# SuperbTUM/Multimodal-ReID

Hardware: AMD Instinct MI355X
Metric: gallery imgs/sec + eval wall-sec (distmat+rerank); mAP parity Market/MSMT17 (higher is better)
Workload: dtype fp16; 1 GPU; Market-1501 full eval: 3368q x 15913g, ViT-B/16 stride-12 (211 tokens), 2 passes/img (plain + flip/pad/crop TTA), exact-fp32 distmat, CMC/mAP; batch=20480, images_per_encoder_call=19281, parallelism=dp1 (image shards + all-gather)

## Files before the change

### include/reidmi_tools.h

```cpp
#ifndef REIDMI_TOOLS_H
#define REIDMI_TOOLS_H
#include "reidmi.h"

#ifdef __cplusplus
extern "C" {
#endif

int reidmi_distmat_f32_variant(const float* q, int64_t Q, int64_t ldq, const float* g, int64_t G, int64_t ldg,
                               int64_t D, float* out, int64_t ldo, float* ws, int variant, void* stream);

int64_t reidmi_search_ex_workspace_bytes(int64_t Q, int64_t G, int64_t D, int k, int splits, int cap);
int reidmi_search_f32_ex(const float* q, int64_t Q, int64_t ldq, const float* g, int64_t G, int64_t ldg, int64_t D,
                         int k, const int64_t* q_pids, const int64_t* q_cams, const int64_t* g_pids,
                         const int64_t* g_cams, int32_t* out_idx, float* out_dist, int64_t ldo, void* ws,
                         int64_t ws_bytes, int splits, int cap, int32_t* stats, void* stream);
int reidmi_search_bounded_f32_ex(const float* q, int64_t Q, int64_t ldq, const float* g, int64_t G, int64_t ldg,
                                 int64_t D, int k, const int64_t* q_pids, const int64_t* q_cams,
                                 const int64_t* g_pids, const int64_t* g_cams, const float* bound_dist,
                                 const int32_t* bound_idx, int64_t ldb, int64_t index_base, int32_t* out_idx,
                                 float* out_dist, int64_t ldo, void* ws, int64_t ws_bytes, int splits, int cap,
                                 int32_t* stats, void* stream);

int reidmi_gemm_f16_tiled(int epi, const void* A, int64_t lda, const void* W, int64_t ldw, int64_t M, int64_t N,
                          int64_t K, const float* bias, const void* rowstat, const float* colsum, void* out,
                          int64_t ldc, int tile, int ngroups, void* stream);

int reidmi_gemm_f16_w4(const void* A, int64_t lda, const void* W, int64_t ldw, int64_t M, int64_t N, int64_t K,
                       const float* bias, void* out, int64_t ldc, int nostore, void* stream);

int reidmi_mhsa_f16_rr(const void* q, const void* k, const void* vt, void* o, int64_t nseq, int L, int H,
                       void* stream);

int reidmi_mhsa_cls_f16(const void* q, const void* k, const void* vt, void* o, int64_t nseq, int L, int H,
                        void* stream);

int reidmi_mhsa_cls_long_f16(const void* q, const void* k, const void* vt, void* o, int64_t nseq, int L, int H,
                             void* stream);

int64_t reidmi_cls_attn_nokv_ws_bytes(int64_t nseq, int W);
int reidmi_cls_attn_nokv_f16(const void* x, const void* rs, const void* q, const void* wqkv, const float* colsum,
// ... 30 lines not shown
```

### multimodal-reid_amd/csrc/encoder.hip

```cpp
#include "attention.h"
#include "gemm.h"

namespace reidmi {

template <typename TX>
__device__ __forceinline__ float4 load4(const TX* p) {
    if constexpr (sizeof(TX) == 4) {
        return *(const float4*)p;
    } else {
        const f16x4 h = *(const f16x4*)p;
        return make_float4((float)h[0], (float)h[1], (float)h[2], (float)h[3]);
    }
}

template <int NV, typename TX>
__global__ __launch_bounds__(256) void layernorm_kernel(const TX* x, int64_t rows, int64_t ldx,
                                                        const int32_t* __restrict__ row_idx,
                                                        const float* __restrict__ gamma,
                                                        const float* __restrict__ beta, float eps,
                                                        float* __restrict__ y32, int64_t ldy32,
                                                        _Float16* __restrict__ y16, int64_t ldy16,
                                                        _Float16* yh, int64_t ldyh, float2* __restrict__ st,
                                                        float2* __restrict__ sto) {
    const int64_t r = (int64_t)blockIdx.x * 4 + (threadIdx.x >> 6);
// ... 369 lines not shown
    int64_t x, h, q, k, vt, o, u, rows, st, st_cls, pst, total;
};

static int64_t al(int64_t v) { return (v + 255) & ~(int64_t)255; }

static Plan plan(int64_t nseq, int L, int W, int lp, int64_t extra_rows) {
    Plan p{};
    const int64_t M = nseq * L;
    int64_t off = 0;
    p.x = off; off = al(off + M * W * 2);
    p.h = off; off = al(off + M * W * 2);
    p.q = off; off = al(off + M * W * 2);
    p.k = off; off = al(off + M * W * 2);
    p.vt = off; off = al(off + nseq * W * (int64_t)lp * 2);
    p.o = off; off = al(off + M * W * 2);
    p.u = off; off = al(off + M * 4 * W * 2);
    p.rows = off; off = al(off + extra_rows * 4);
    p.st = off; off = al(off + (M + 256) * 8);
    p.st_cls = off; off = al(off + (nseq + 256) * 8);
    p.pst = off; off = al(off + M * (W / 64) * 8);
    p.total = off;
    return p;
}

enum XStats { XS_ROWS = 0, XS_PARTIALS = 1, XS_READY = 2 };

static int ln1_stats(XStats xs, char* ws, const Plan& P, int64_t M, int W, hipStream_t s) {
    float2* st = (float2*)(ws + P.st);
    if (xs == XS_READY) return OK;
    if (xs == XS_PARTIALS) return row_stats_from_partials((const float2*)(ws + P.pst), M, W, st, s);
    return row_stats((const _Float16*)(ws + P.x), M, W, W, st, s);
}

static int run_block(const reidmi_block_weights& bw, char* ws, const Plan& P, int64_t nseq, int L, int W, int H,
                     bool causal, XStats xs, hipStream_t s) {
    const int64_t M = nseq * L;
    float2* pst = (float2*)(ws + P.pst);
    _Float16* x = (_Float16*)(ws + P.x);
    _Float16* o = (_Float16*)(ws + P.o);
    _Float16* u = (_Float16*)(ws + P.u);
    float2* st = (float2*)(ws + P.st);
    int rc;
    if ((rc = ln1_stats(xs, ws, P, M, W, s))) return rc;
    {
        EpiArgs ea{};
        ea.bias = bw.qkv_b;
        ea.rowstat = st;
        ea.colsum = bw.qkv_s;
        ea.q = ws + P.q;
        ea.k = ws + P.k;
        ea.vt = ws + P.vt;
// ... 5 lines not shown
    }
    EpiArgs er{};
    er.out = x;
    er.ldc = W;
    er.bias = bw.out_b;
    er.pstat = pst;
    er.ldp = M;
    if ((rc = gemm_f16(EPI_RESID_F16, o, W, bw.out_w, W, M, W, W, er, s))) return rc;
    if ((rc = row_stats_from_partials(pst, M, W, st, s))) return rc;
    EpiArgs eg{};
    eg.out = u;
    eg.ldc = 4 * W;
    eg.bias = bw.fc1_b;
    eg.rowstat = st;
    eg.colsum = bw.fc1_s;
    if ((rc = gemm_f16(EPI_GELU_H16, x, W, bw.fc1_w, W, M, 4 * W, W, eg, s))) return rc;
    EpiArgs e2{};
    e2.out = x;
    e2.ldc = W;
    e2.bias = bw.fc2_b;
    e2.pstat = pst;
    e2.ldp = M;
    if ((rc = gemm_f16(EPI_RESID_F16, u, 4 * W, bw.fc2_w, 4 * W, M, W, 4 * W, e2, s))) return rc;
    return OK;
}

__global__ void gather_rowstat_kernel(const float2* __restrict__ st, int64_t nseq, int L, float2* __restrict__ sc) {
    const int64_t b = (int64_t)blockIdx.x * blockDim.x + threadIdx.x;
    if (b < nseq) sc[b] = st[b * L];
}

static int run_block_cls(const reidmi_block_weights& bw, char* ws, const Plan& P, int64_t nseq, int L, int W, int H,
                         XStats xs, hipStream_t s) {
    const int64_t M = nseq * L;
    _Float16* x = (_Float16*)(ws + P.x);
    _Float16* o = (_Float16*)(ws + P.o);
    _Float16* u = (_Float16*)(ws + P.u);
    float2* st = (float2*)(ws + P.st);
// ... 69 lines not shown

REIDMI_API int reidmi_layernorm(const float* x, int64_t rows, int64_t ldx, const int32_t* row_idx, int64_t W,
                                const float* gamma, const float* beta, float eps, float* y32, int64_t ldy32, void* y16,
                                int64_t ldy16, void* stream) {
    return layernorm(x, rows, ldx, row_idx, W, gamma, beta, eps, y32, ldy32, (_Float16*)y16, ldy16,
                     (hipStream_t)stream);
}

REIDMI_API int64_t reidmi_vit_workspace_bytes(const reidmi_vit_weights* w, int64_t B, int full) {
    if (vit_check(w)) return -1;
    const int64_t L = 1 + (int64_t)w->grid_h * w->grid_w + w->n_ctx;
    if (L < 1 || L > kAttnLongMax) return -1;
    return plan(B, (int)L, w->width, attn_vt_stride((int)L), 0).total;
}

REIDMI_API int reidmi_vit_forward(const reidmi_vit_weights* w, const void* images, int images_f16, int64_t B, int H,
                                  int Wimg, const int32_t* tta, int full, float* out_x12, float* out_proj,
                                  float* out_x11, void* ws_, int64_t ws_bytes, void* stream) {
    int rc;
    if ((rc = vit_check(w))) return rc;
    hipStream_t s = (hipStream_t)stream;
    RM_REQUIRE(1 + (int64_t)w->grid_h * w->grid_w + w->n_ctx <= 1024, "vit: too many tokens (max 1024)");
    const int W = w->width, NP = w->grid_h * w->grid_w, L = 1 + NP + w->n_ctx, E = w->out_dim;
    RM_REQUIRE((H - w->patch) / w->stride + 1 == w->grid_h && (Wimg - w->patch) / w->stride + 1 == w->grid_w,
               "vit: image size does not match the positional-embedding grid");
    const Plan P = plan(B, L, W, attn_vt_stride(L), 0);
    RM_REQUIRE(ws_bytes >= P.total, "vit: workspace too small");
    RM_REQUIRE(out_x12 && out_proj, "vit: outputs required");
    if (B == 0) return OK;
    char* ws = (char*)ws_;
    _Float16* x = (_Float16*)(ws + P.x);
    _Float16* h = (_Float16*)(ws + P.h);
    _Float16* col = (_Float16*)(ws + P.u);
    const int64_t M = B * L;
    if ((rc = im2col(images, images_f16, B, H, Wimg, w->patch, w->stride, w->grid_h, w->grid_w, w->kpad, tta, col, s)))
        return rc;
    if ((rc = patch_embed(col, w->conv_w, w->pos_emb, w->class_emb, w->vpt, w->n_ctx, B, NP, W, w->kpad, x, s)))
        return rc;
    if ((rc = layernorm(x, M, W, nullptr, W, w->ln_pre_w, w->ln_pre_b, 1e-5f, nullptr, 0, nullptr, 0, s, x, W, nullptr,
                        (float2*)(ws + P.st))))
        return rc;
    for (int i = 0; i < 12; i++) {
        const reidmi_block_weights& bw = w->blocks[i];
        if (i > 0 && bw.prompt && w->n_ctx > 0) {
            const int64_t pe = B * w->n_ctx * W;
            hipLaunchKernelGGL(prompt_rows_kernel, dim3(ceil_div(pe, 256)), dim3(256), 0, s, x, B, L, W,
                               L - w->n_ctx, w->n_ctx, bw.prompt);
            RM_LAUNCHED();
        }
        const XStats xs = i == 0 ? XS_READY : (bw.prompt && w->n_ctx > 0) ? XS_ROWS : XS_PARTIALS;
        if (i == 11 && !full) rc = run_block_cls(bw, ws, P, B, L, W, w->heads, xs, s);
        else rc = run_block(bw, ws, P, B, L, W, w->heads, false, xs, s);
        if (rc) return rc;
        if (i == 10 && out_x11) {
            const int64_t r11 = full ? M : B;
            hipLaunchKernelGGL(rows_f16_to_f32_kernel, dim3(ceil_div(r11 * (W / 4), 256)), dim3(256), 0, s, x, r11,
                               full ? (int64_t)W : (int64_t)L * W, W, out_x11);
            RM_LAUNCHED();
        }
    }
    const int64_t rows = full ? M : B;
    const int64_t ldx = full ? W : (int64_t)L * W;
    if ((rc = layernorm(x, rows, ldx, nullptr, W, w->ln_post_w, w->ln_post_b, 1e-5f, out_x12, W, h, W, s))) return rc;
    EpiArgs eo{};
    eo.out = out_proj;
    eo.ldc = E;
    if ((rc = gemm_f16(EPI_F32, h, W, w->proj_t, W, rows, E, W, eo, s))) return rc;
    return OK;
}

REIDMI_API int64_t reidmi_text_workspace_bytes(const reidmi_text_weights* w, int64_t N) {
    if (!w || attn_lpad(w->ctx) < 0) return -1;
    return plan(N, w->ctx, w->width, attn_lpad(w->ctx), N).total;
}

REIDMI_API int reidmi_text_forward(const reidmi_text_weights* w, const int64_t* tokens, const float* prompts,
                                   int64_t N, int ctx_used, float* out, void* ws_, int64_t ws_bytes, void* stream) {
    RM_REQUIRE(w && w->blocks && tokens && out, "text: null argument");
    RM_REQUIRE(w->width == w->heads * 64 && w->width % 256 == 0, "text: width");
    hipStream_t s = (hipStream_t)stream;
    const int W = w->width, Lt = w->ctx, E = w->out_dim;
    const int L = ctx_used > 0 ? ctx_used : Lt;
    RM_REQUIRE(L <= Lt && L > w->n_ctx, "text: ctx_used must be in (n_ctx, ctx]");
    RM_REQUIRE(attn_lpad(L) > 0, "text: context too long");
    const Plan P = plan(N, L, W, attn_lpad(L), N);
    RM_REQUIRE(ws_bytes >= P.total, "text: workspace too small");
    if (N == 0) return OK;
    char* ws = (char*)ws_;
    _Float16* x = (_Float16*)(ws + P.x);
    _Float16* h = (_Float16*)(ws + P.h);
    int32_t* rows = (int32_t*)(ws + P.rows);
    int rc;
    if ((rc = text_embed(x, tokens, prompts, w->tok_emb, w->pos_emb, N, L, Lt, W, (int64_t)w->vocab, s))) return rc;
    for (int i = 0; i < w->layers; i++) {
        const reidmi_block_weights& bw = w->blocks[i];
        if (i > 0 && bw.prompt && w->n_ctx > 0) {
            const int64_t pe = N * w->n_ctx * W;
            hipLaunchKernelGGL(prompt_rows_kernel, dim3(ceil_div(pe, 256)), dim3(256), 0, s, x, N, L, W, 1,
                               w->n_ctx, bw.prompt);
            RM_LAUNCHED();
        }
        const XStats xs = i > 0 && !(bw.prompt && w->n_ctx > 0) ? XS_PARTIALS : XS_ROWS;
        if ((rc = run_block(bw, ws, P, N, L, W, w->heads, true, xs, s))) return rc;
    }
    if ((rc = eot_rows(tokens, N, L, Lt, rows, s))) return rc;
    if ((rc = layernorm(x, N, W, rows, W, w->ln_final_w, w->ln_final_b, 1e-5f, nullptr, 0, h, W, s))) return rc;
    EpiArgs eo{};
    eo.out = out;
// ... 11 lines not shown
REIDMI_API int reidmi_gemm_f16_resid_partials(const void* A, int64_t lda, const void* Wt, int64_t ldw, int64_t M,
                                              int64_t N, int64_t K, const float* bias, void* out, int64_t ldc,
                                              void* pst, void* stream) {
    RM_REQUIRE(A && Wt && out && pst && N % 64 == 0, "resid partials: null argument or N % 64 != 0");
    EpiArgs e{};
    e.out = out;
    e.ldc = ldc;
    e.bias = bias;
    e.pstat = (float2*)pst;
    e.ldp = M;
    return gemm_f16(EPI_RESID_F16, (const _Float16*)A, lda, (const _Float16*)Wt, ldw, M, (int)N, (int)K, e,
                    (hipStream_t)stream);
}

#ifdef REIDMI_TOOLS
REIDMI_API int reidmi_im2col_f16(const void* images, int images_f16, int64_t B, int H, int Wimg, int patch, int stride,
                                 int gh, int gw, int kpad, const int32_t* tta, void* col, void* stream) {
    RM_REQUIRE(images && col && B >= 0 && H > 0 && Wimg > 0, "im2col: null argument or bad shape");
    return im2col(images, images_f16, B, H, Wimg, patch, stride, gh, gw, kpad, tta, (_Float16*)col,
                  (hipStream_t)stream);
}

REIDMI_API int reidmi_patch_embed_f16(const void* col, const void* conv_w, const float* pos_emb,
                                      const float* class_emb, const float* vpt, int n_ctx, int64_t B, int NP, int W,
                                      int kpad, void* x, int tile, void* stream) {
    RM_REQUIRE(col && conv_w && pos_emb && class_emb && x && n_ctx >= 0 && B >= 0 && NP > 0 && W > 0,
               "patch_embed: null argument or bad shape");
    if (B == 0) return OK;
    GemmOpts opt;
    opt.tile = tile;
// ... 25 lines not shown
```

### multimodal-reid_amd/csrc/gemm.h

```cpp
#pragma once
#include "common.h"

namespace reidmi {

enum Epi : int {
    EPI_H16 = 0,
    EPI_GELU_H16 = 1,
    EPI_QKV = 3,
    EPI_PATCH = 4,
    EPI_F32 = 5,
    EPI_RESID_F16 = 6,
    EPI_RRHI = 7,
    EPI_RRSV = 8
};

struct EpiArgs {
    void* out;
    int64_t ldc;
    const float* bias;
    void* q;
    void* k;
    void* vt;
    int seq;
    int heads;
// ... 11 lines not shown
    int64_t rr_n;
    float rr_c[3];
    const float* rr_csqn;
    const float* rr_cnrm;
    const float4* rr_rowmeta;
    const float4* rr_colrec;
    const int* rr_tiles;
    int64_t rr_ntiles;
    int rr_tri;
    int* sv_cnt;
    int2* sv_list;
    int sv_cap;
    const float* dist_rsq;
    const float* dist_csq;
    int64_t dist_n;
};

__device__ __forceinline__ float rr_hi(float dot, float si, float sj, float crn_i, float ni, float nj,
                                       const float (&c)[3]) {
    const float s = si + sj;
    const float dt = __builtin_fmaf(-2.0f, dot, s);
    const float e = 1.01f * (__builtin_fmaf(crn_i, nj, 0x1p-23f * s) + c[1] * (ni + nj) + c[2]);
    return dt + e;
}

struct GemmOpts {
    int tile = 0;
    int ngroups = 0;
    int band = -1;
};

int gemm_f16(int epi, const void* A, int64_t lda, const void* W, int64_t ldw, int64_t M, int64_t N, int64_t K,
             const EpiArgs& ea, hipStream_t stream, const GemmOpts& opts = GemmOpts{});

int gemm_api(int epi, const void* A, int64_t lda, const void* W, int64_t ldw, int64_t M, int64_t N, int64_t K,
             const float* bias, const void* rowstat, const float* colsum, void* out, int64_t ldc, const GemmOpts& opt,
             void* stream);

int prof_begin(double flops, int epi, hipStream_t s, hipEvent_t* end);
int prof_end(hipEvent_t end, hipStream_t s);

}
```

### multimodal-reid_amd/csrc/gemm.hip

```cpp
#include "gemm_epilogue.h"
#include "gemm_rrsv.h"
#include <type_traits>

namespace reidmi {

template <int EPI>
__global__ __launch_bounds__(256, 2) void gemm_tile_kernel(const _Float16* __restrict__ A, int64_t lda,
                                                           const _Float16* __restrict__ W, int64_t ldw, int64_t M,
                                                           int N, int K, EpiArgs ea, int tiles_n, int nwg) {
    __shared__ __attribute__((aligned(16))) _Float16 smem[2][2][GB_M * GB_K];
    const int bid = blockIdx.x;
    const int xcd = bid & 7, qq = nwg >> 3, rr = nwg & 7;
    const int wg = (xcd < rr ? xcd * (qq + 1) : rr * (qq + 1) + (xcd - rr) * qq) + (bid >> 3);
    const int tm = wg / tiles_n, tn = wg % tiles_n;
    const int64_t m0 = (int64_t)tm * GB_M;
    const int n0 = tn * GB_N;
    const int tid = threadIdx.x, lane = tid & 63, wid = tid >> 6;
    const int wm = wid >> 1, wn = wid & 1;

    const _Float16* gA[4];
    const _Float16* gW[4];
    int soff[4];
    bool aval[4];
#pragma unroll
// ... 66 lines not shown
        const int cq = (lane >> 4) * 4;
#pragma unroll
        for (int j = 0; j < 4; j++)
            bn[j] = ea.bias ? *(const float4*)(ea.bias + n0 + wn * 64 + j * 16 + cq) : make_float4(0.f, 0.f, 0.f, 0.f);
        ln_fold<4>(acc, ea.rowstat, ea.colsum, bn, m0 + wm * 64, n0 + wn * 64, M);
        epilogue_tile<EPI, 4, true>(ea, acc, m0 + wm * 64, n0 + wn * 64, M, N);
        return;
    }
    epilogue_tile<EPI, 4>(ea, acc, m0 + wm * 64, n0 + wn * 64, M, N);
#undef GLOAD
#undef LSTORE
}

constexpr int G2_STAGE = (G2_M + G2_N) * GB_K;

template <int EPI, int TAG = 0>
__global__ __launch_bounds__(512, 2) void gemm_persistent_kernel(const _Float16* __restrict__ A, int64_t lda,
                                                                 const _Float16* __restrict__ W, int64_t ldw,
                                                                 int64_t M, int N, int K, EpiArgs ea, int tiles_m,
                                                                 int tiles_n, int ngroups, int band) {
    extern __shared__ __attribute__((aligned(16))) _Float16 lds[];
    const int G = gridDim.x;
    const int bid = blockIdx.x;
    const int ng = G < 8 ? G : 8;
    const int xg = bid % ng, gx = G / ng + ((G % ng) > xg ? 1 : 0);
    const int ngr = (ng == 8 && 8 % ngroups == 0 && ngroups <= tiles_n) ? ngroups : 1;
    const int xper = ng / ngr, grp = xg / xper, xs = xg - grp * xper;
    const int nb0 = tiles_n * grp / ngr, tnk = tiles_n * (grp + 1) / ngr - nb0;
    const int64_t sub = (int64_t)tiles_m * tnk;
    const int lo = (int)(sub * xs / xper), hi = (int)(sub * (xs + 1) / xper);
    const int first = lo + bid / ng;
    if (first >= hi) return;
    if constexpr (EPI == EPI_RESID_F16) {
        if (bid & 1) __builtin_amdgcn_s_sleep(127);
    }
    const int tid = threadIdx.x, lane = tid & 63;
    const int wid = __builtin_amdgcn_readfirstlane(tid >> 6);
    const int wr = wid >> 2, wc = wid & 3;
    const int nk = K / GB_K;

    int rowA[2][2], kcA[2][2], offA[2][2], offW[2][2];
    uint32_t offAb[2][2], offWb[2][2];
#pragma unroll
    for (int h = 0; h < 2; h++)
#pragma unroll
        for (int u = 0; u < 2; u++) {
            const int pc = 2 * wid + u;
            const int ra = 128 * (pc >> 3) + 64 * h + 8 * (pc & 7);
            const int rb = 64 * (pc >> 2) + 32 * h + 8 * (pc & 3);
            const int r1 = ra + (lane >> 3), r2 = rb + (lane >> 3);
            rowA[h][u] = r1;
            kcA[h][u] = ((lane & 7) ^ ((r1 >> 1) & 7)) * 8;
            offAb[h][u] = (uint32_t)(r1 * (int)lda + kcA[h][u]) * 2u;
            offWb[h][u] = (uint32_t)(r2 * (int)ldw + ((lane & 7) ^ ((r2 >> 1) & 7)) * 8) * 2u;
            offA[h][u] = ra * GB_K;
            offW[h][u] = G2_M * GB_K + rb * GB_K;
        }
    const int* const rr_list = EPI == EPI_RRSV ? ea.rr_tiles : nullptr;
    if constexpr (EPI != EPI_RRHI) band = 0;
    struct Pos {
        int tile, kt;
        int64_t m0;
        int n0;
        bool full;
        const char* a;
        const char* w;
    };
    auto set_tile = [&](Pos& p, int tile) {
        p.tile = tile;
        p.kt = 0;
        int mt, nt;
        tile_mn<EPI == EPI_RRSV>(tile, tnk, band, tiles_m, rr_list, mt, nt);
        p.m0 = (int64_t)mt * G2_M;
        p.n0 = (nb0 + nt) * G2_N;
        p.full = p.m0 + G2_M <= M;
        p.a = (const char*)(A + (GEMM_VAR_ASAME ? 0 : p.m0) * lda);
        p.w = (const char*)(W + (int64_t)p.n0 * ldw);
    };
    auto advance = [&](Pos& p) {
        if (++p.kt == nk) {
            set_tile(p, p.tile + gx);
        } else {
            p.a += GB_K * 2;
            p.w += GB_K * 2;
        }
    };
    auto issue_a = [&](int stage, int h, const Pos& p) {
        const char* base = p.a;
        if (p.full) {
#pragma unroll
            for (int u = 0; u < 2; u++)
                __builtin_amdgcn_global_load_lds(base + offAb[h][u],
                                                 (lds_ptr_t)(lds + stage * G2_STAGE + offA[h][u]), 16, 0, 0);
        } else {
            const int lim = (int)(M - p.m0);
#pragma unroll
            for (int u = 0; u < 2; u++) {
                const int r = rowA[h][u] < lim ? rowA[h][u] : lim - 1;
                __builtin_amdgcn_global_load_lds(base + (uint32_t)(r * (int)lda + kcA[h][u]) * 2u,
                                                 (lds_ptr_t)(lds + stage * G2_STAGE + offA[h][u]), 16, 0, 0);
            }
        }
    };
    auto issue_w = [&](int stage, int h, const Pos& p) {
// ... 212 lines not shown
#pragma unroll
            for (int i = 0; i < 8; i++)
#pragma unroll
                for (int j = 0; j < 4; j++) {
                    acc[i][j][0] = __builtin_fmaf(rs[i].x, acc[i][j][0], __builtin_fmaf(rs[i].y, sn[j].x, b[j].x));
                    acc[i][j][1] = __builtin_fmaf(rs[i].x, acc[i][j][1], __builtin_fmaf(rs[i].y, sn[j].y, b[j].y));
                    acc[i][j][2] = __builtin_fmaf(rs[i].x, acc[i][j][2], __builtin_fmaf(rs[i].y, sn[j].z, b[j].z));
                    acc[i][j][3] = __builtin_fmaf(rs[i].x, acc[i][j][3], __builtin_fmaf(rs[i].y, sn[j].w, b[j].w));
                }
        }
        if constexpr (EPI == EPI_RRSV)
            rrsv_tile(ea, acc, m0 + wr * 128, n0 + wc * 64, M, seq, ea.rr_tri && tmt < tnt, rr_lds + (seq & 1) * 4096,
                      rr_lds + 8192 + (seq & 1) * 4096, sv_lds, sv_n, lane,
                      RrsvWalk{first, gx, wr, wc, rr_list});
        else if (EPI == EPI_GELU_H16 && m0 + G2_M <= M)
            epilogue_tile<EPI, 8, true, RPRE, true>(ea, acc, m0 + wr * 128, n0 + wc * 64, M, N, xres);
        else
            epilogue_tile<EPI, 8, true, RPRE>(ea, acc, m0 + wr * 128, n0 + wc * 64, M, N, xres);
        seq++;
        if (wr == 1) G5_BARRIER();
    }
    if constexpr (EPI == EPI_RRSV)
        rrsv_flush(ea, sv_lds, sv_n, lane, RrsvWalk{first, gx, wr, wc, rr_list});
    if (wr == 0) G5_BARRIER();
#undef G5_BARRIER
#undef G5_LDS_DONE
}

template <int EPI>
static int launch(const void* A, int64_t lda, const void* W, int64_t ldw, int64_t M, int64_t N, int64_t K,
                  const EpiArgs& ea, hipStream_t s, const GemmOpts& opt) {
    const bool listed = EPI == EPI_RRSV;
    RM_REQUIRE(!listed || (ea.rr_tiles && ea.rr_ntiles > 0), "gemm: the survivor epilogue needs its tile list");
    const int64_t tiles256 = listed ? ea.rr_ntiles : (int64_t)ceil_div(M, G2_M) * (N / G2_N);
    const bool fits = N % G2_N == 0 && K >= 2 * GB_K && lda * G2_M < (1ll << 31) && ldw * G2_N < (1ll << 31);
    if (fits && (opt.tile == 2 || (opt.tile == 0 && tiles256 >= 256))) {
        const int tiles_m = listed ? (int)tiles256 : ceil_div(M, G2_M), tiles_n = listed ? 1 : (int)(N / G2_N);
        RM_REQUIRE(tiles256 < (1ll << 31), "gemm: grid too large");
        RM_REQUIRE(!listed || (ceil_div(M, G2_M) <= 65536 && N / G2_N <= 65536), "gemm: tile list: too many tiles");
        RM_REQUIRE(EPI != EPI_RRSV || tiles256 / (tiles256 < 256 ? tiles256 : 256) < (1 << 18),
                   "gemm: survivor epilogue: too many tiles per workgroup");
        const size_t lds = 2 * (size_t)G2_STAGE * 2 + (EPI == EPI_RRSV ? kRrsvSlotBytes : 3 * 8 * 256 * sizeof(float));
        const bool tag1 = EPI == EPI_RESID_F16 && K > N;
        auto kern = tag1 ? gemm_persistent_kernel<EPI, EPI == EPI_RESID_F16 ? 1 : 0> : gemm_persistent_kernel<EPI, 0>;
        static bool attr[2] = {false, false};
        if (!attr[tag1]) {
            RM_CHECK_HIP(hipFuncSetAttribute((const void*)kern, hipFuncAttributeMaxDynamicSharedMemorySize, (int)lds));
            attr[tag1] = true;
        }
        const int grid = (int)(tiles256 < 256 ? tiles256 : 256);
        const int ngroups =
            listed ? 1 : opt.ngroups > 0 ? opt.ngroups : (tiles_n % 2 == 0 && tiles_n >= 8 ? 2 : 1);
        const int band = EPI != EPI_RRHI ? 0 : opt.band >= 0 ? opt.band : RR_GEMM_BAND;
        hipLaunchKernelGGL(kern, dim3((unsigned)grid), dim3(512), lds, s, (const _Float16*)A,
                           lda, (const _Float16*)W, ldw, M, (int)N, (int)K, ea, tiles_m, tiles_n, ngroups, band);
        RM_LAUNCHED();
        return OK;
    }
    if constexpr (EPI == EPI_RRSV) {
        return fail(EINVAL_, "gemm: the survivor epilogue runs on the persistent 256 x 256 tile only "
                             "(N % 256 == 0, K >= 128, >= 256 tiles)");
    } else {
    const int tiles_m = ceil_div(M, GB_M), tiles_n = (int)(N / GB_N);
    const int64_t nwg = (int64_t)tiles_m * tiles_n;
    RM_REQUIRE(nwg < (1ll << 31), "gemm: grid too large");
    hipLaunchKernelGGL((gemm_tile_kernel<EPI>), dim3((unsigned)nwg), dim3(256), 0, s, (const _Float16*)A, lda,
                       (const _Float16*)W, ldw, M, (int)N, (int)K, ea, tiles_n, (int)nwg);
    RM_LAUNCHED();
    return OK;
    }
}

int gemm_f16(int epi, const void* A, int64_t lda, const void* W, int64_t ldw, int64_t M, int64_t N, int64_t K,
// ... 3 lines not shown
    RM_REQUIRE(opt.ngroups == 0 || opt.ngroups == 1 || opt.ngroups == 2 || opt.ngroups == 4 || opt.ngroups == 8,
               "gemm walk: ngroups in {0 (auto), 1, 2, 4, 8}");
    RM_REQUIRE(M >= 0 && N > 0 && K > 0, "gemm: bad shape");
    RM_REQUIRE((epi != EPI_QKV && epi != EPI_PATCH) || M < (1ll << 31), "gemm: head split / patch rows need M < 2^31");
    RM_REQUIRE(N % GB_N == 0 && K % GB_K == 0, "gemm: needs N % 128 == 0 and K % 64 == 0");
    RM_REQUIRE(lda % 8 == 0 && ldw % 8 == 0 && lda >= K && ldw >= K, "gemm: lda/ldw must be >= K and 16-byte rows");
    RM_REQUIRE((epi != EPI_H16 && epi != EPI_GELU_H16 && epi != EPI_RESID_F16) ||
                   (ea.ldc % 8 == 0 && ((uintptr_t)ea.out & 15) == 0 && ea.ldc < (1 << 24) && N < (1 << 24)),
               "gemm: fp16 output needs ldc % 8 == 0 (< 2^24) and a 16-byte aligned base");
    RM_REQUIRE((ea.rowstat == nullptr) == (ea.colsum == nullptr), "gemm: rowstat and colsum go together");
    RM_REQUIRE(ea.rowstat == nullptr || ea.bias != nullptr, "gemm: a folded LayerNorm needs the folded bias");
    RM_REQUIRE(epi != EPI_RESID_F16 || ea.rowstat == nullptr, "gemm: the residual epilogue takes no folded LayerNorm");
    RM_REQUIRE(ea.dist_rsq == nullptr || (epi == EPI_F32 && ea.dist_csq != nullptr && ea.dist_n > 0 &&
                                          ea.dist_n <= N && ea.ldc >= ea.dist_n && ea.bias == nullptr),
               "gemm: the distance form needs EPI_F32, both norm vectors, 0 < dist_n <= N, ldc >= dist_n, no bias");
    if (M == 0) return OK;
    hipEvent_t ev_b = nullptr;
    if (const int prc = prof_begin(2.0 * (double)M * (double)N * (double)K, epi, s, &ev_b)) return prc;
    int rc;
    switch (epi) {
        case EPI_H16: rc = launch<EPI_H16>(A, lda, W, ldw, M, N, K, ea, s, opt); break;
        case EPI_GELU_H16: rc = launch<EPI_GELU_H16>(A, lda, W, ldw, M, N, K, ea, s, opt); break;
        case EPI_QKV: rc = launch<EPI_QKV>(A, lda, W, ldw, M, N, K, ea, s, opt); break;
        case EPI_PATCH: rc = launch<EPI_PATCH>(A, lda, W, ldw, M, N, K, ea, s, opt); break;
        case EPI_F32: rc = launch<EPI_F32>(A, lda, W, ldw, M, N, K, ea, s, opt); break;
        case EPI_RESID_F16: rc = launch<EPI_RESID_F16>(A, lda, W, ldw, M, N, K, ea, s, opt); break;
        case EPI_RRHI: rc = launch<EPI_RRHI>(A, lda, W, ldw, M, N, K, ea, s, opt); break;
        case EPI_RRSV: rc = launch<EPI_RRSV>(A, lda, W, ldw, M, N, K, ea, s, opt); break;
        default: return fail(EINVAL_, "gemm: unknown epilogue");
    }
// ... 29 lines not shown
```

### multimodal-reid_amd/csrc/gemm_epilogue.h

```cpp
#pragma once
#include "gemm.h"

namespace reidmi {

constexpr int GB_M = 128, GB_N = 128, GB_K = 64;
constexpr int G2_M = 256, G2_N = 256;
typedef __attribute__((address_space(3))) void* lds_ptr_t;

#ifndef GEMM_VAR_NOSTORE
#define GEMM_VAR_NOSTORE 0
#endif
#ifndef GEMM_VAR_NOGELU
#define GEMM_VAR_NOGELU 0
#endif
#ifndef GEMM_VAR_NOPSTAT
#define GEMM_VAR_NOPSTAT 0
#endif
#ifndef GEMM_VAR_NORESLOAD
#define GEMM_VAR_NORESLOAD 0
#endif
#ifndef GEMM_VAR_NODMA
#define GEMM_VAR_NODMA 0
#endif
#ifndef GEMM_VAR_NOWAIT
// ... 72 lines not shown
    const int lane = threadIdx.x & 63, q = lane >> 4;
    const int64_t b0 = mrow < M ? mrow : M - 1;
    const char* const ob = (const char*)((const _Float16*)ea.out + b0 * ea.ldc);
#pragma unroll
    for (int i = 0; i < NI; i++) {
        int64_t m = mrow + i * 16 + (lane & 15);
        m = m < M ? m : M - 1;
#pragma unroll
        for (int jp = 0; jp < 2; jp++) {
            const int c = ncol + (2 * jp + (q & 1)) * 16 + (q >> 1) * 8;
            xv[i][jp] = *(const f16x8*)(ob + (uint32_t)((int)(m - b0) * (int)ea.ldc + c) * 2u);
        }
    }
}

template <int EPI, int NI, bool BIAS_DONE = false, bool PRE = false, bool FULL = false>
__device__ __forceinline__ void epilogue_tile(const EpiArgs& ea, f32x4 (&acc)[NI][4], int64_t mrow, int ncol,
                                              int64_t M, int N, const f16x8 (*xpre)[2] = nullptr) {
    const int lane = threadIdx.x & 63;
    const int cq = (lane >> 4) * 4;
    [[maybe_unused]] const int64_t b0 = mrow < M ? mrow : M - 1;
    [[maybe_unused]] char* const ob = (char*)((_Float16*)ea.out + b0 * ea.ldc);
    [[maybe_unused]] auto obo = [&](int64_t m, int c) -> uint32_t {
        return (uint32_t)((int)(m - b0) * (int)ea.ldc + c) * 2u;
    };
    if (!BIAS_DONE && EPI != EPI_PATCH && ea.bias != nullptr) {
        float4 b[4];
#pragma unroll
        for (int j = 0; j < 4; j++) b[j] = *(const float4*)(ea.bias + ncol + j * 16 + cq);
#pragma unroll
        for (int i = 0; i < NI; i++)
// ... 258 lines not shown
#pragma unroll
                for (int j = 0; j < 4; j++) {
                    const f32x4 v = acc[i][j];
                    const int hd = qkv_c0 + j * 16 + cq;
                    _Float16* dst = vb + (int64_t)hd * lp;
                    dst[0] = (_Float16)v[0];
                    dst[lp] = (_Float16)v[1];
                    dst[2 * lp] = (_Float16)v[2];
                    dst[3 * lp] = (_Float16)v[3];
                }
            }
            return;
        }
    }
    const int q = lane >> 4;
#pragma unroll
    for (int i = 0; i < NI; i++) {
        const int64_t m = mrow + i * 16 + (lane & 15);
        [[maybe_unused]] _Float16* qkrow = nullptr;
        if constexpr (EPI == EPI_QKV) {
            const uint32_t seq = (uint32_t)ea.seq;
            const uint32_t b = (uint32_t)m / seq, t = (uint32_t)m - b * seq;
            qkrow = (_Float16*)(qkv_sel == 0 ? ea.q : ea.k) + ((int64_t)b * ea.heads * ea.seq + t) * 64;
        }
#pragma unroll
        for (int jp = 0; jp < 2; jp++) {
            f32x4 a = acc[i][2 * jp], c = acc[i][2 * jp + 1];
            if constexpr (EPI == EPI_GELU_H16 && !GEMM_VAR_NOGELU) {
#pragma unroll
                for (int e = 0; e < 4; e += 2) {
// ... 6 lines not shown
                }
            }
            const auto lo = __builtin_amdgcn_permlane16_swap(cvt_pk_f16(a[0], a[1]), cvt_pk_f16(c[0], c[1]), false, false);
            const auto hi = __builtin_amdgcn_permlane16_swap(cvt_pk_f16(a[2], a[3]), cvt_pk_f16(c[2], c[3]), false, false);
            const uint4 v = make_uint4(lo[0], hi[0], lo[1], hi[1]);
            const int col = ncol + (2 * jp + (q & 1)) * 16 + (q >> 1) * 8;
            if (!FULL && m >= M) continue;
            if constexpr (EPI == EPI_QKV) {
                const int hd = qkv_c0 + (col - ncol);
                *(uint4*)(qkrow + (int64_t)(hd >> 6) * ea.seq * 64 + (hd & 63)) = v;
            } else {
                if constexpr (GEMM_VAR_NOSTORE) {
                    typedef unsigned u32x4v __attribute__((ext_vector_type(4)));
                    asm volatile("" ::"v"(__builtin_bit_cast(u32x4v, v)));
                }
                else *(uint4*)(ob + obo(m, col)) = v;
            }
        }
    }
}

template <int EPI>
struct EpiVm {
    static constexpr int count = EPI == EPI_H16 || EPI == EPI_GELU_H16 || EPI == EPI_QKV ? 16
                                 : EPI == EPI_RESID_F16 || EPI == EPI_F32 || EPI == EPI_RRHI ? 32
                                                                                          : -1;
};

}
```

### multimodal-reid_amd/csrc/gemm_tools.hip

```cpp
#ifdef REIDMI_TOOLS
#include "gemm_epilogue.h"

#ifndef W4_VAR_NODMA
#define W4_VAR_NODMA 0
#endif
#ifndef W4_VAR_NOWAIT
#define W4_VAR_NOWAIT 0
#endif
#ifndef W4_VAR_NOBARRIER
#define W4_VAR_NOBARRIER 0
#endif
namespace reidmi {
template <bool NOSTORE>
__global__ __launch_bounds__(256) __attribute__((amdgpu_waves_per_eu(1, 1))) void gemm_w4_kernel(
    const _Float16* __restrict__ A, int64_t lda, const _Float16* __restrict__ W, int64_t ldw, int64_t M, int N, int K,
    EpiArgs ea, int tiles_n, int ntiles) {
    extern __shared__ __attribute__((aligned(16))) _Float16 lds[];
    constexpr int STAGE = (G2_M + G2_N) * GB_K;
    const int lane = threadIdx.x & 63;
    const int wid = __builtin_amdgcn_readfirstlane(threadIdx.x >> 6);
    const int wr = wid >> 1, wc = wid & 1;
    const int nk = K / GB_K;
    const int G = gridDim.x;
    const bool isA = wid < 2;
// ... 125 lines not shown
    hipLaunchKernelGGL(kern, dim3((unsigned)grid), dim3(256), lds, (hipStream_t)stream, (const _Float16*)A, lda,
                       (const _Float16*)W, ldw, M, (int)N, (int)K, ea, tiles_n, (int)ntiles);
    RM_LAUNCHED();
    return OK;
}

REIDMI_API int reidmi_gemm_f16_tiled(int epi, const void* A, int64_t lda, const void* W, int64_t ldw, int64_t M,
                                     int64_t N, int64_t K, const float* bias, const void* rowstat, const float* colsum,
                                     void* out, int64_t ldc, int tile, int ngroups, void* stream) {
    GemmOpts opt;
    opt.tile = tile;
    opt.ngroups = ngroups;
    return gemm_api(epi, A, lda, W, ldw, M, N, K, bias, rowstat, colsum, out, ldc, opt, stream);
}

static int qkv_api(const void* A, int64_t lda, const void* W, int64_t ldw, int64_t nseq, int L, int H, int64_t N,
                   int64_t n_off, const float* bias, const void* rowstat, const float* colsum, void* q, void* k,
                   void* vt, int lpad, const GemmOpts& opt, void* stream) {
    const int64_t wd = (int64_t)H * 64;
    RM_REQUIRE(nseq >= 0 && L > 0 && H > 0 && lpad >= L, "gemm_f16_qkv: bad shape");
    RM_REQUIRE(N > 0 && n_off >= 0 && n_off % 64 == 0 && n_off + N <= 3 * wd, "gemm_f16_qkv: columns outside [q | k | v]");
    RM_REQUIRE((q || n_off >= wd) && (k || n_off >= 2 * wd || n_off + N <= wd) && (vt || n_off + N <= 2 * wd),
               "gemm_f16_qkv: null output for a produced column block");
    EpiArgs ea{};
    ea.bias = bias;
    ea.rowstat = (const float2*)rowstat;
    ea.colsum = colsum;
    ea.q = q;
    ea.k = k;
    ea.vt = vt;
// ... 25 lines not shown
```

Before: 13490 imgs/s.

## Store MLP hidden activations in pre-swizzled 256x64 blocks for c_proj loads

```diff
diff --git a/include/reidmi_tools.h b/include/reidmi_tools.h
--- a/include/reidmi_tools.h
+++ b/include/reidmi_tools.h
@@ -24,6 +24,14 @@
 int reidmi_gemm_f16_tiled(int epi, const void* A, int64_t lda, const void* W, int64_t ldw, int64_t M, int64_t N,
                           int64_t K, const float* bias, const void* rowstat, const float* colsum, void* out,
                           int64_t ldc, int tile, int ngroups, void* stream);
+
+int reidmi_mlp_pair_f16(void* x, const void* fc1_w, const float* fc1_b, const void* rowstat, const float* fc1_s,
+                        const void* fc2_w, const float* fc2_b, int64_t M, int W, void* u, int64_t u_bytes, void* pst,
+                        int blocked, int which, int tile, void* stream);
+
+int reidmi_vit_forward_ex(const reidmi_vit_weights* w, const void* images, int images_f16, int64_t B, int H, int Wimg,
+                          const int32_t* tta, int full, float* out_x12, float* out_proj, float* out_x11, void* ws,
+                          int64_t ws_bytes, int mlp_blocked, void* stream);
 
 int reidmi_gemm_f16_w4(const void* A, int64_t lda, const void* W, int64_t ldw, int64_t M, int64_t N, int64_t K,
                        const float* bias, void* out, int64_t ldc, int nostore, void* stream);
diff --git a/multimodal-reid_amd/csrc/encoder.hip b/multimodal-reid_amd/csrc/encoder.hip
--- a/multimodal-reid_amd/csrc/encoder.hip
+++ b/multimodal-reid_amd/csrc/encoder.hip
@@ -407,7 +407,7 @@
     p.k = off; off = al(off + M * W * 2);
     p.vt = off; off = al(off + nseq * W * (int64_t)lp * 2);
     p.o = off; off = al(off + M * W * 2);
-    p.u = off; off = al(off + M * 4 * W * 2);
+    p.u = off; off = al(off + u_blocked_elems(M, 4 * (int64_t)W) * 2);
     p.rows = off; off = al(off + extra_rows * 4);
     p.st = off; off = al(off + (M + 256) * 8);
     p.st_cls = off; off = al(off + (nseq + 256) * 8);
@@ -426,8 +426,9 @@
 }
 
 static int run_block(const reidmi_block_weights& bw, char* ws, const Plan& P, int64_t nseq, int L, int W, int H,
-                     bool causal, XStats xs, hipStream_t s) {
+                     bool causal, XStats xs, hipStream_t s, bool blocked_ok = true) {
     const int64_t M = nseq * L;
+    const bool ublk = blocked_ok && mlp_u_blocked(M, W);
     float2* pst = (float2*)(ws + P.pst);
     _Float16* x = (_Float16*)(ws + P.x);
     _Float16* o = (_Float16*)(ws + P.o);
@@ -463,6 +464,7 @@
     eg.bias = bw.fc1_b;
     eg.rowstat = st;
     eg.colsum = bw.fc1_s;
+    eg.out_blocked = ublk;
     if ((rc = gemm_f16(EPI_GELU_H16, x, W, bw.fc1_w, W, M, 4 * W, W, eg, s))) return rc;
     EpiArgs e2{};
     e2.out = x;
@@ -470,7 +472,16 @@
     e2.bias = bw.fc2_b;
     e2.pstat = pst;
     e2.ldp = M;
-    if ((rc = gemm_f16(EPI_RESID_F16, u, 4 * W, bw.fc2_w, 4 * W, M, W, 4 * W, e2, s))) return rc;
+    GemmOpts o2;
+    o2.a_blocked = ublk;
+    if ((rc = gemm_f16(EPI_RESID_F16, u, 4 * W, bw.fc2_w, 4 * W, M, W, 4 * W, e2, s, o2))) return rc;
+    return OK;
+}
+
+static int zero_u_pad(char* ws, const Plan& P, int64_t M, int W, hipStream_t s, bool blocked_ok = true) {
+    if (!blocked_ok || M % 256 == 0 || !mlp_u_blocked(M, W)) return OK;
+    const int64_t tile_bytes = 256 * 4 * (int64_t)W * 2;
+    RM_CHECK_HIP(hipMemsetAsync(ws + P.u + M / 256 * tile_bytes, 0, (size_t)tile_bytes, s));
     return OK;
 }
 
@@ -570,9 +581,9 @@
     return plan(B, (int)L, w->width, attn_vt_stride((int)L), 0).total;
 }
 
-REIDMI_API int reidmi_vit_forward(const reidmi_vit_weights* w, const void* images, int images_f16, int64_t B, int H,
-                                  int Wimg, const int32_t* tta, int full, float* out_x12, float* out_proj,
-                                  float* out_x11, void* ws_, int64_t ws_bytes, void* stream) {
+static int vit_forward(const reidmi_vit_weights* w, const void* images, int images_f16, int64_t B, int H, int Wimg,
+                       const int32_t* tta, int full, float* out_x12, float* out_proj, float* out_x11, void* ws_,
+                       int64_t ws_bytes, void* stream, bool blocked_ok) {
     int rc;
     if ((rc = vit_check(w))) return rc;
     hipStream_t s = (hipStream_t)stream;
@@ -596,6 +607,7 @@
     if ((rc = layernorm(x, M, W, nullptr, W, w->ln_pre_w, w->ln_pre_b, 1e-5f, nullptr, 0, nullptr, 0, s, x, W, nullptr,
                         (float2*)(ws + P.st))))
         return rc;
+    if ((rc = zero_u_pad(ws, P, M, W, s, blocked_ok))) return rc;
     for (int i = 0; i < 12; i++) {
         const reidmi_block_weights& bw = w->blocks[i];
         if (i > 0 && bw.prompt && w->n_ctx > 0) {
@@ -606,7 +618,7 @@
         }
         const XStats xs = i == 0 ? XS_READY : (bw.prompt && w->n_ctx > 0) ? XS_ROWS : XS_PARTIALS;
         if (i == 11 && !full) rc = run_block_cls(bw, ws, P, B, L, W, w->heads, xs, s);
-        else rc = run_block(bw, ws, P, B, L, W, w->heads, false, xs, s);
+        else rc = run_block(bw, ws, P, B, L, W, w->heads, false, xs, s, blocked_ok);
         if (rc) return rc;
         if (i == 10 && out_x11) {
             const int64_t r11 = full ? M : B;
@@ -623,6 +635,13 @@
     eo.ldc = E;
     if ((rc = gemm_f16(EPI_F32, h, W, w->proj_t, W, rows, E, W, eo, s))) return rc;
     return OK;
+}
+
+REIDMI_API int reidmi_vit_forward(const reidmi_vit_weights* w, const void* images, int images_f16, int64_t B, int H,
+                                  int Wimg, const int32_t* tta, int full, float* out_x12, float* out_proj,
+                                  float* out_x11, void* ws_, int64_t ws_bytes, void* stream) {
+    return vit_forward(w, images, images_f16, B, H, Wimg, tta, full, out_x12, out_proj, out_x11, ws_, ws_bytes, stream,
+                       true);
 }
 
 REIDMI_API int64_t reidmi_text_workspace_bytes(const reidmi_text_weights* w, int64_t N) {
@@ -648,6 +667,7 @@
     int32_t* rows = (int32_t*)(ws + P.rows);
     int rc;
     if ((rc = text_embed(x, tokens, prompts, w->tok_emb, w->pos_emb, N, L, Lt, W, (int64_t)w->vocab, s))) return rc;
+    if ((rc = zero_u_pad(ws, P, N * L, W, s))) return rc;
     for (int i = 0; i < w->layers; i++) {
         const reidmi_block_weights& bw = w->blocks[i];
         if (i > 0 && bw.prompt && w->n_ctx > 0) {
@@ -689,6 +709,14 @@
 }
 
 #ifdef REIDMI_TOOLS
+REIDMI_API int reidmi_vit_forward_ex(const reidmi_vit_weights* w, const void* images, int images_f16, int64_t B, int H,
+                                     int Wimg, const int32_t* tta, int full, float* out_x12, float* out_proj,
+                                     float* out_x11, void* ws_, int64_t ws_bytes, int mlp_blocked, void* stream) {
+    RM_REQUIRE(mlp_blocked == 0 || mlp_blocked == 1, "vit_forward_ex: mlp_blocked is 0 or 1");
+    return vit_forward(w, images, images_f16, B, H, Wimg, tta, full, out_x12, out_proj, out_x11, ws_, ws_bytes, stream,
+                       mlp_blocked != 0);
+}
+
 REIDMI_API int reidmi_im2col_f16(const void* images, int images_f16, int64_t B, int H, int Wimg, int patch, int stride,
                                  int gh, int gw, int kpad, const int32_t* tta, void* col, void* stream) {
     RM_REQUIRE(images && col && B >= 0 && H > 0 && Wimg > 0, "im2col: null argument or bad shape");
diff --git a/multimodal-reid_amd/csrc/gemm.h b/multimodal-reid_amd/csrc/gemm.h
--- a/multimodal-reid_amd/csrc/gemm.h
+++ b/multimodal-reid_amd/csrc/gemm.h
@@ -49,7 +49,11 @@
     const float* dist_rsq;
     const float* dist_csq;
     int64_t dist_n;
+    int out_blocked;
 };
+
+constexpr int64_t kUBlockElems = 256 * 64;
+inline int64_t u_blocked_elems(int64_t M, int64_t K) { return (M + 255) / 256 * 256 * K; }
 
 __device__ __forceinline__ float rr_hi(float dot, float si, float sj, float crn_i, float ni, float nj,
                                        const float (&c)[3]) {
@@ -63,7 +67,15 @@
     int tile = 0;
     int ngroups = 0;
     int band = -1;
+    int a_blocked = 0;
 };
+
+bool gemm_is_persistent(int64_t M, int64_t N, int64_t K, int64_t lda, int64_t ldw, const GemmOpts& opts = GemmOpts{});
+
+inline bool mlp_u_blocked(int64_t M, int W, const GemmOpts& opts = GemmOpts{}) {
+    return gemm_is_persistent(M, 4 * (int64_t)W, W, W, W, opts) &&
+           gemm_is_persistent(M, W, 4 * (int64_t)W, 4 * (int64_t)W, 4 * (int64_t)W, opts);
+}
 
 int gemm_f16(int epi, const void* A, int64_t lda, const void* W, int64_t ldw, int64_t M, int64_t N, int64_t K,
              const EpiArgs& ea, hipStream_t stream, const GemmOpts& opts = GemmOpts{});
diff --git a/multimodal-reid_amd/csrc/gemm.hip b/multimodal-reid_amd/csrc/gemm.hip
--- a/multimodal-reid_amd/csrc/gemm.hip
+++ b/multimodal-reid_amd/csrc/gemm.hip
@@ -104,7 +104,7 @@
 
 constexpr int G2_STAGE = (G2_M + G2_N) * GB_K;
 
-template <int EPI, int TAG = 0>
+template <int EPI, int TAG = 0, bool BLK = false>
 __global__ __launch_bounds__(512, 2) void gemm_persistent_kernel(const _Float16* __restrict__ A, int64_t lda,
                                                                  const _Float16* __restrict__ W, int64_t ldw,
                                                                  int64_t M, int N, int K, EpiArgs ea, int tiles_m,
@@ -128,6 +128,9 @@
     const int wid = __builtin_amdgcn_readfirstlane(tid >> 6);
     const int wr = wid >> 2, wc = wid & 3;
     const int nk = K / GB_K;
+    constexpr bool ABLK = BLK && EPI == EPI_RESID_F16;
+    constexpr bool CBLK = BLK && EPI == EPI_GELU_H16;
+    static_assert(!BLK || ABLK || CBLK, "blocked u: c_fc's output or c_proj's A only");
 
     int rowA[2][2], kcA[2][2], offA[2][2], offW[2][2];
     uint32_t offAb[2][2], offWb[2][2];
@@ -141,7 +144,7 @@
             const int r1 = ra + (lane >> 3), r2 = rb + (lane >> 3);
             rowA[h][u] = r1;
             kcA[h][u] = ((lane & 7) ^ ((r1 >> 1) & 7)) * 8;
-            offAb[h][u] = (uint32_t)(r1 * (int)lda + kcA[h][u]) * 2u;
+            offAb[h][u] = ABLK ? (uint32_t)(ra * GB_K * 2 + lane * 16) : (uint32_t)(r1 * (int)lda + kcA[h][u]) * 2u;
             offWb[h][u] = (uint32_t)(r2 * (int)ldw + ((lane & 7) ^ ((r2 >> 1) & 7)) * 8) * 2u;
             offA[h][u] = ra * GB_K;
             offW[h][u] = G2_M * GB_K + rb * GB_K;
@@ -164,20 +167,23 @@
         p.m0 = (int64_t)mt * G2_M;
         p.n0 = (nb0 + nt) * G2_N;
         p.full = p.m0 + G2_M <= M;
-        p.a = (const char*)(A + (GEMM_VAR_ASAME ? 0 : p.m0) * lda);
+        if constexpr (ABLK)
+            p.a = (const char*)(A + (GEMM_VAR_ASAME ? 0 : (int64_t)mt) * nk * kUBlockElems);
+        else
+            p.a = (const char*)(A + (GEMM_VAR_ASAME ? 0 : p.m0) * lda);
         p.w = (const char*)(W + (int64_t)p.n0 * ldw);
     };
     auto advance = [&](Pos& p) {
         if (++p.kt == nk) {
             set_tile(p, p.tile + gx);
         } else {
-            p.a += GB_K * 2;
+            p.a += ABLK ? kUBlockElems * 2 : GB_K * 2;
             p.w += GB_K * 2;
         }
     };
     auto issue_a = [&](int stage, int h, const Pos& p) {
         const char* base = p.a;
-        if (p.full) {
+        if (ABLK || p.full) {
 #pragma unroll
             for (int u = 0; u < 2; u++)
                 __builtin_amdgcn_global_load_lds(base + offAb[h][u],
@@ -420,9 +426,9 @@
                       rr_lds + 8192 + (seq & 1) * 4096, sv_lds, sv_n, lane,
                       RrsvWalk{first, gx, wr, wc, rr_list});
         else if (EPI == EPI_GELU_H16 && m0 + G2_M <= M)
-            epilogue_tile<EPI, 8, true, RPRE, true>(ea, acc, m0 + wr * 128, n0 + wc * 64, M, N, xres);
+            epilogue_tile<EPI, 8, true, RPRE, true, CBLK>(ea, acc, m0 + wr * 128, n0 + wc * 64, M, N, xres);
         else
-            epilogue_tile<EPI, 8, true, RPRE>(ea, acc, m0 + wr * 128, n0 + wc * 64, M, N, xres);
+            epilogue_tile<EPI, 8, true, RPRE, false, CBLK>(ea, acc, m0 + wr * 128, n0 + wc * 64, M, N, xres);
         seq++;
         if (wr == 1) G5_BARRIER();
     }
@@ -431,6 +437,17 @@
     if (wr == 0) G5_BARRIER();
 #undef G5_BARRIER
 #undef G5_LDS_DONE
+}
+
+static bool persistent_fits(int64_t N, int64_t K, int64_t lda, int64_t ldw) {
+    return N % G2_N == 0 && K >= 2 * GB_K && lda * G2_M < (1ll << 31) && ldw * G2_N < (1ll << 31);
+}
+static bool persistent_chosen(int64_t tiles256, const GemmOpts& opt) {
+    return opt.tile == 2 || (opt.tile == 0 && tiles256 >= 256);
+}
+
+bool gemm_is_persistent(int64_t M, int64_t N, int64_t K, int64_t lda, int64_t ldw, const GemmOpts& opt) {
+    return persistent_fits(N, K, lda, ldw) && persistent_chosen((int64_t)ceil_div(M, G2_M) * (N / G2_N), opt);
 }
 
 template <int EPI>
@@ -439,8 +456,8 @@
     const bool listed = EPI == EPI_RRSV;
     RM_REQUIRE(!listed || (ea.rr_tiles && ea.rr_ntiles > 0), "gemm: the survivor epilogue needs its tile list");
     const int64_t tiles256 = listed ? ea.rr_ntiles : (int64_t)ceil_div(M, G2_M) * (N / G2_N);
-    const bool fits = N % G2_N == 0 && K >= 2 * GB_K && lda * G2_M < (1ll << 31) && ldw * G2_N < (1ll << 31);
-    if (fits && (opt.tile == 2 || (opt.tile == 0 && tiles256 >= 256))) {
+    const bool blk = (EPI == EPI_GELU_H16 && ea.out_blocked) || (EPI == EPI_RESID_F16 && opt.a_blocked);
+    if (persistent_fits(N, K, lda, ldw) && persistent_chosen(tiles256, opt)) {
         const int tiles_m = listed ? (int)tiles256 : ceil_div(M, G2_M), tiles_n = listed ? 1 : (int)(N / G2_N);
         RM_REQUIRE(tiles256 < (1ll << 31), "gemm: grid too large");
         RM_REQUIRE(!listed || (ceil_div(M, G2_M) <= 65536 && N / G2_N <= 65536), "gemm: tile list: too many tiles");
@@ -448,11 +465,14 @@
                    "gemm: survivor epilogue: too many tiles per workgroup");
         const size_t lds = 2 * (size_t)G2_STAGE * 2 + (EPI == EPI_RRSV ? kRrsvSlotBytes : 3 * 8 * 256 * sizeof(float));
         const bool tag1 = EPI == EPI_RESID_F16 && K > N;
-        auto kern = tag1 ? gemm_persistent_kernel<EPI, EPI == EPI_RESID_F16 ? 1 : 0> : gemm_persistent_kernel<EPI, 0>;
-        static bool attr[2] = {false, false};
-        if (!attr[tag1]) {
+        constexpr bool CAN_BLK = EPI == EPI_GELU_H16 || EPI == EPI_RESID_F16;
+        auto kern = tag1 ? (blk ? gemm_persistent_kernel<EPI, EPI == EPI_RESID_F16 ? 1 : 0, CAN_BLK>
+                                : gemm_persistent_kernel<EPI, EPI == EPI_RESID_F16 ? 1 : 0>)
+                         : (blk ? gemm_persistent_kernel<EPI, 0, EPI == EPI_GELU_H16> : gemm_persistent_kernel<EPI, 0>);
+        static bool attr[2][2] = {{false, false}, {false, false}};
+        if (!attr[tag1][blk]) {
             RM_CHECK_HIP(hipFuncSetAttribute((const void*)kern, hipFuncAttributeMaxDynamicSharedMemorySize, (int)lds));
-            attr[tag1] = true;
+            attr[tag1][blk] = true;
         }
         const int grid = (int)(tiles256 < 256 ? tiles256 : 256);
         const int ngroups =
@@ -463,6 +483,7 @@
         RM_LAUNCHED();
         return OK;
     }
+    if (blk) return fail(EINVAL_, "gemm: a blocked MLP hidden buffer needs the persistent 256 x 256 tile");
     if constexpr (EPI == EPI_RRSV) {
         return fail(EINVAL_, "gemm: the survivor epilogue runs on the persistent 256 x 256 tile only "
                              "(N % 256 == 0, K >= 128, >= 256 tiles)");
@@ -496,6 +517,10 @@
     RM_REQUIRE(ea.dist_rsq == nullptr || (epi == EPI_F32 && ea.dist_csq != nullptr && ea.dist_n > 0 &&
                                           ea.dist_n <= N && ea.ldc >= ea.dist_n && ea.bias == nullptr),
                "gemm: the distance form needs EPI_F32, both norm vectors, 0 < dist_n <= N, ldc >= dist_n, no bias");
+    RM_REQUIRE(!ea.out_blocked || (epi == EPI_GELU_H16 && ea.ldc == N && N % GB_K == 0),
+               "gemm: a blocked output is c_fc's (EPI_GELU_H16) with ldc == N");
+    RM_REQUIRE(!opt.a_blocked || (epi == EPI_RESID_F16 && lda == K && K > N),
+               "gemm: a blocked A is c_proj's (EPI_RESID_F16, K > N) with lda == K");
     if (M == 0) return OK;
     hipEvent_t ev_b = nullptr;
     if (const int prc = prof_begin(2.0 * (double)M * (double)N * (double)K, epi, s, &ev_b)) return prc;
diff --git a/multimodal-reid_amd/csrc/gemm_epilogue.h b/multimodal-reid_amd/csrc/gemm_epilogue.h
--- a/multimodal-reid_amd/csrc/gemm_epilogue.h
+++ b/multimodal-reid_amd/csrc/gemm_epilogue.h
@@ -110,7 +110,7 @@
     }
 }
 
-template <int EPI, int NI, bool BIAS_DONE = false, bool PRE = false, bool FULL = false>
+template <int EPI, int NI, bool BIAS_DONE = false, bool PRE = false, bool FULL = false, bool BLK = false>
 __device__ __forceinline__ void epilogue_tile(const EpiArgs& ea, f32x4 (&acc)[NI][4], int64_t mrow, int ncol,
                                               int64_t M, int N, const f16x8 (*xpre)[2] = nullptr) {
     const int lane = threadIdx.x & 63;
@@ -399,6 +399,14 @@
         }
     }
     const int q = lane >> 4;
+    [[maybe_unused]] char* ub = nullptr;
+    [[maybe_unused]] uint32_t uo = 0;
+    if constexpr (BLK) {
+        static_assert(EPI == EPI_GELU_H16 && NI == 8, "blocked u: c_fc's epilogue on the persistent tile");
+        const int r = lane & 15;
+        ub = (char*)ea.out + (((mrow >> 8) * (ea.ldc >> 6) + (ncol >> 6)) * kUBlockElems + (mrow & 255) * GB_K) * 2;
+        uo = (uint32_t)(r * 128 + (((2 * (q & 1) + (q >> 1)) ^ ((r >> 1) & 7)) << 4));
+    }
 #pragma unroll
     for (int i = 0; i < NI; i++) {
         const int64_t m = mrow + i * 16 + (lane & 15);
@@ -435,6 +443,7 @@
                     typedef unsigned u32x4v __attribute__((ext_vector_type(4)));
                     asm volatile("" ::"v"(__builtin_bit_cast(u32x4v, v)));
                 }
+                else if constexpr (BLK) *(uint4*)(ub + ((uo ^ (uint32_t)(jp << 6)) + (uint32_t)(i * 2048))) = v;
                 else *(uint4*)(ob + obo(m, col)) = v;
             }
         }
diff --git a/multimodal-reid_amd/csrc/gemm_tools.hip b/multimodal-reid_amd/csrc/gemm_tools.hip
--- a/multimodal-reid_amd/csrc/gemm_tools.hip
+++ b/multimodal-reid_amd/csrc/gemm_tools.hip
@@ -163,6 +163,40 @@
     return gemm_api(epi, A, lda, W, ldw, M, N, K, bias, rowstat, colsum, out, ldc, opt, stream);
 }
 
+REIDMI_API int reidmi_mlp_pair_f16(void* x, const void* fc1_w, const float* fc1_b, const void* rowstat,
+                                   const float* fc1_s, const void* fc2_w, const float* fc2_b, int64_t M, int W, void* u,
+                                   int64_t u_bytes, void* pst, int blocked, int which, int tile, void* stream) {
+    RM_REQUIRE(x && fc1_w && fc2_w && u && M > 0 && W > 0, "mlp_pair: null argument or bad shape");
+    RM_REQUIRE((blocked == 0 || blocked == 1) && which >= 0 && which <= 2, "mlp_pair: blocked is 0 or 1, which 0..2");
+    const int64_t N4 = 4 * (int64_t)W;
+    RM_REQUIRE(u_bytes >= (blocked ? u_blocked_elems(M, N4) : M * N4) * 2, "mlp_pair: u too small");
+    GemmOpts opt;
+    opt.tile = tile;
+    RM_REQUIRE(!blocked || mlp_u_blocked(M, W, opt), "mlp_pair: the blocked buffer needs the persistent tile on both GEMMs");
+    int rc;
+    if (which != 2) {
+        EpiArgs eg{};
+        eg.out = u;
+        eg.ldc = N4;
+        eg.bias = fc1_b;
+        eg.rowstat = (const float2*)rowstat;
+        eg.colsum = fc1_s;
+        eg.out_blocked = blocked;
+        if ((rc = gemm_f16(EPI_GELU_H16, x, W, fc1_w, W, M, N4, W, eg, (hipStream_t)stream, opt))) return rc;
+    }
+    if (which != 1) {
+        EpiArgs e2{};
+        e2.out = x;
+        e2.ldc = W;
+        e2.bias = fc2_b;
+        e2.pstat = (float2*)pst;
+        e2.ldp = M;
+        opt.a_blocked = blocked;
+        if ((rc = gemm_f16(EPI_RESID_F16, u, N4, fc2_w, N4, M, W, N4, e2, (hipStream_t)stream, opt))) return rc;
+    }
+    return OK;
+}
+
 static int qkv_api(const void* A, int64_t lda, const void* W, int64_t ldw, int64_t nseq, int L, int H, int64_t N,
                    int64_t n_off, const float* bias, const void* rowstat, const float* colsum, void* q, void* k,
                    void* vt, int lpad, const GemmOpts& opt, void* stream) {
```

Measured after the change: 13510 imgs/s (median of 2 runs). Within noise of the previous version (+0.1%).
